# slobodaapl/nvit

Measured on AMD Instinct MI355X. Metric: images/sec (train step) nViT-B/16 224px, higher is better.
Workload: dtype bf16; 1 GPU; nViT-base 224px patches 8/16 T=784 C=768 L=12 H=12, full train step (fwd+bwd+clip+AdamW+renorm), synthetic images, formula weights; per_gpu_batch=128, global_batch=128, parallelism=dp1

## Files before the change

include/nvit_hip.h:

```cpp
#ifndef NVIT_HIP_H
#define NVIT_HIP_H
#include <stdint.h>

#ifdef __cplusplus
extern "C" {
#endif

#define NVIT_OK 0
#define NVIT_EINVAL 1001
#define NVIT_F32 0
#define NVIT_BF16 1
#define NVIT_BF16_F32IN 3

int nvit_version(void);
const char* nvit_last_error(void);

#define NVIT_KID_GEMM_NT 0
#define NVIT_KID_GEMM_TN 1
#define NVIT_KID_ATTN_FWD 2
#define NVIT_KID_ATTN_BWD 3
#define NVIT_KID_ROWOPS 4
#define NVIT_KID_RENORM 5
#define NVIT_KID_SHADOW 6
#define NVIT_KID_PATCHIFY 7
#define NVIT_KID_MISC 8
#define NVIT_KID_GEMM_F32 9
#define NVIT_KID_GEMM_SWIGLU 10
#define NVIT_KID_GEMM_QKNORM 11
#define NVIT_KID_GEMM_SWIGLU_BWD 12
#define NVIT_KID_OPTIM 13
#define NVIT_KID_GEMM_SWIGLU_ACT 14
#define NVIT_KID_COUNT 15
void nvit_prof_enable(int on);
void nvit_prof_select(unsigned mask);
int nvit_prof_collect(double* ms, double* flops, double* bytes, int64_t* launches);
const char* nvit_prof_name(int kid);

#define NVIT_RENORM_ROWS_PER_ITEM 64
#define NVIT_RENORM_COLS_PER_ITEM 64
#define NVIT_RENORM_TALL_ROWS 1152
#define NVIT_RENORM_TALL_COLS_PER_ITEM 32
#define NVIT_RENORM_MAX_ROWS_DIM0 2048
int nvit_renorm_weights(const int64_t* table, int n, int total_items, void* stream);

int nvit_shadow_weights(const int64_t* table, int n, int total_items, int dt, void* stream);

int nvit_adamw_tick(float* hyper, double beta1, double beta2, void* stream);
int nvit_grad_sqnorm(const int64_t* table, int n, int total_chunks, float* partial, int npart, void* stream);
int nvit_adamw_renorm(const int64_t* table, int n, int total_items, int max_slab_rows, float beta1, float beta2,
                      float eps, double bias_correction1, double bias_correction2, const float* partial, int npart,
                      float max_norm, float* gnorm_out, const float* hyper, void* stream);

int nvit_gemm_nt(int dt, const void* A, int lda, const void* B, int ldb, void* C, int ldc, int out_dt,
                 int M, int N, int K, const float* bias, const float* colscale, const float* rowadd,
                 int rowadd_period, int accumulate, void* stream);

int nvit_set_gemm_sched(int dynamic);
int nvit_set_gemm_impl(int nt_impl, int tn_impl);
int nvit_gemm_nt_fusable(int dt, int M, int N, int K);
int nvit_gemm_nt_swiglu_bwd(int dt, const void* A, int lda, const void* B, int ldb, const void* uv, void* duv,
                            float* part, int M, int F, int K, const float* gs, float gscale, void* stream);
int nvit_gemm_nt_swiglu(int dt, const void* A, int lda, const void* B, int ldb, void* uv, void* xm, int M, int F,
                        int K, const float* gs, float gscale, void* stream);
int nvit_gemm_nt_swiglu_act(int dt, const void* A, int lda, const void* B, int ldb, void* xm, int M, int F, int K,
                            const float* gs, float gscale, void* stream);
int nvit_gemm_nt_qknorm(int dt, const void* A, int lda, const void* B, int ldb, int M, int K, int nparts, int part0,
                        const float* sqk, float c_q, float q_prescale, void* qh, void* kh, void* vh, float* rq, float* rk,
                        int T, int H, int d, void* stream);
int nvit_gemm_nt_swiglu_bias(int dt, const void* A, int lda, const void* B, int ldb, void* uv, void* xm, int M, int F,
                             int K, const float* gs, float gscale, const float* bias, void* stream);
int nvit_gemm_nt_swiglu_act_bias(int dt, const void* A, int lda, const void* B, int ldb, void* xm, int M, int F, int K,
                                 const float* gs, float gscale, const float* bias, void* stream);
int nvit_gemm_nt_qknorm_bias(int dt, const void* A, int lda, const void* B, int ldb, int M, int K, int nparts, int part0,
                             const float* sqk, float c_q, float q_prescale, void* qh, void* kh, void* vh, float* rq,
                             float* rk, int T, int H, int d, const float* bias, void* stream);

int nvit_gemm_tn(int dt, const void* A, int lda, const void* B, int ldb, float* G, int ldg, int Mred, int N,
                 int K, int splits, float* ws, int64_t ws_bytes, int perm, int accumulate, void* stream);

int nvit_lerp_fwd(int dt, const float* h, const void* y, int y_dt, const float* alpha, float c_a,
                  const float* skip_x, const float* skip, float* out, void* out_lo, int M, int C, void* stream);
int nvit_lerp_bwd_blocks(int dt, int y_dt, int C, int has_add, int has_skip, int accum);
int nvit_lerp_bwd(int dt, const float* dout, const void* dout_add, const float* h, const void* y, int y_dt, const float* alpha,
                  float c_a, const float* skip_x, const float* skip, float* dh, int accum_dh, float* dy,
                  void* dy_lo, float* dskip_x, float* part_dlam, float* part_dskip, int nblk, int M, int C,
                  void* stream);

int nvit_rmsnorm_fwd(const float* x, const float* w, float eps, float* out, float* rstd, int M, int C, void* stream);
int nvit_rmsnorm_bwd(const float* dout, const float* x, const float* w, const float* rstd, float* dx, float* part_dw,
                     int nblk, int M, int C, void* stream);
int nvit_res_rmsnorm_fwd(int dt, const float* a, const void* y, int y_dt, const float* w, float eps, float* out,
                         void* out_lo, float* rstd, int M, int C, void* stream);
int nvit_res_rmsnorm_bwd(int dt, const float* g, const void* g_add, const float* a, const void* y, int y_dt,
                         const float* w, const float* rstd, float* dz, int accum, void* dz_lo, float* part_dw, int nblk,
                         int M, int C, void* stream);
int nvit_res_skip_fwd(int dt, const float* h, const void* y, int y_dt, const float* skip, const float* x, float* out,
                      void* out_lo, int M, int C, void* stream);
int nvit_res_skip_bwd(int dt, const float* dout, const float* h, const void* y, int y_dt, const float* skip,
                      const float* x, float* dh, void* dh_lo, float* dx, float* part_dskip, int nblk, int M, int C,
                      void* stream);
int nvit_norm_skip_fwd(const float* src, const float* tgt, const float* skip, float* out, int M, int C, void* stream);
int nvit_norm_skip_bwd(const float* dout, const float* src, const float* tgt, const float* skip, float* dsrc,
                       float* dtgt, float* part_dskip, int nblk, int M, int C, void* stream);

int nvit_qknorm_fwd(int dt, const void* q, int ldq, const void* k, int ldk, const void* v, int ldv,
                    const float* sqk, float c_q, void* qh, void* kh, void* vh, float* rq, float* rk, int B,
                    int T, int H, int d, void* stream);
int nvit_qknorm_bwd(int dt, const void* dqh, const void* dkh, const void* dvh, const void* qh, const void* kh,
                    const float* rq, const float* rk, const float* sqk, float c_q, void* dq, int ldq,
                    void* dk, int ldk, void* dv, int ldv, float* part_dsqk, int nblk, int B, int T, int H,
                    int d, void* stream);

int nvit_heads_pad_fwd(int dt, const float* q, int ldq, const float* k, int ldk, const float* v, int ldv,
                       const float* sqk, float c_q, void* qh, void* kh, void* vh, float* rq, float* rk,
                       float* sqk_pad, int B, int T, int H, int d, int dp, void* stream);
int nvit_heads_pad_bwd(int dt, const void* dqh, const void* dkh, const void* dvh, const void* qh, const void* kh,
                       const float* rq, const float* rk, const float* sqk, float c_q, void* dq, int ldq,
                       void* dk, int ldk, void* dv, int ldv, float* part_dsqk, int nblk, int B, int T, int H,
                       int d, int dp, void* stream);
int nvit_pad_cols(int dt, const void* src, void* dst, int M, int H, int d, int dp, void* stream);
int nvit_unpad_cols(int dt, const void* src, void* dst, int M, int H, int d, int dp, void* stream);

int nvit_swiglu_fwd(int dt, const void* uv, const float* suv, float gscale, void* x, int M, int F, void* stream);
int nvit_swiglu_bwd(int dt, const void* dx, const void* uv, const float* suv, float gscale, void* duv,
                    float* part_dsuv, int rows_per_blk, int M, int F, void* stream);

int nvit_colsum_reduce(const float* part, int nblk, int N, float* out, int accumulate, int kind, const float* ref,
                       float scale, void* stream);
int nvit_colsum_reduce_multi(const int64_t* part, const int* nblk, const int64_t* part_b, const int* nblk_b, const int* N,
                             const int64_t* out, const int* accumulate, const int* kind, const int64_t* ref,
                             const float* scale, int n, void* stream);
int nvit_colsum(const void* a, int a_dt, int lda, const void* b, int b_dt, int ldb, int R, int N, int period,
                float* out, int accumulate, float scale, void* stream);
int nvit_cast(const float* src, void* dst, int dt, int64_t n, void* stream);
int nvit_normalize_images(const void* in, int in_is_u8_hwc, float* out, int B, int C, int H, int W, float mean, float std_,
                          void* stream);
int nvit_scale_cols(const float* a, int lda, const float* s, float c, void* out, int out_dt, int ldo, int R, int N,
                    void* stream);

int nvit_attn_fwd(int dt, int impl, const void* qh, const void* kh, const void* vh, float scale, void* o, float* lse,
                  int B, int H, int Tq, int Tk, int d, void* stream);
int nvit_attn_fwd_bounded(int dt, int impl, const void* qh, const void* kh, const void* vh, float scale, const float* sqk,
                          float c_q, float q_prescale, void* o, float* lse, int B, int H, int Tq, int Tk, int d,
                          void* stream);
int nvit_attn_bwd(int dt, int impl, const void* dout, const void* qh, const void* kh, const void* vh, const void* o,
                  const float* lse, float scale, void* dqh, void* dkh, void* dvh, float* delta, int B, int H,
                  int Tq, int Tk, int d, void* stream);

int nvit_attn_bwd_qknorm(int dt, const void* dout, const void* qh, const void* kh, const void* vh, const void* o,
                         const float* lse, float scale, const float* rq, const float* rk, const float* sqk, float c_q,
                         float q_prescale, void* dq, int ldq, void* dk, void* dv, int ldkv, float* part_q, float* part_k,
                         float* delta, int B, int H, int Tq, int Tk, int d, void* stream);

#define NVIT_ATTN_HEADS_MAX_H 32
int nvit_attn_heads_fwd(int dt, const float* q, int ldq, const float* k, const float* v, int ldkv, const float* sqk,
                        float c_q, float scale, void* o, float* lse, int M, int H, int d, void* stream);
int nvit_attn_heads_bwd(int dt, const void* dout, const float* q, int ldq, const float* k, const float* v, int ldkv,
                        const float* sqk, float c_q, float scale, const float* lse, void* dq, int lddq, void* dk,
                        void* dv, int lddkv, float* part_dsqk, int nblk, int M, int H, int d, void* stream);

int nvit_im2col(int dt, const float* img, void* A_l, void* A_g, int B, int ch, int S, int Pl, int Pg, void* stream);
int nvit_patch_embed_kp(int K);
int nvit_patch_embed_fwd(const float* img, const void* w_l, const float* b_l, const float* pos_l, float* out_l, void* lo_l,
                         void* a_l, const void* w_g, const float* b_g, const float* pos_g, float* out_g, void* lo_g,
                         void* a_g, int B, int ch, int S, int Pl, int Pg, int C, void* stream);
int nvit_pool_ln_fwd(int dt, const float* x, const float* w, const float* b, float eps, float* pooled, float* ln,
                     void* ln_lo, float* stats, float* ws, int nchunk, int B, int T, int C, void* stream);
int nvit_pool_ln_bwd(const float* dln, const float* pooled, const float* w, const float* stats, float* dx,
                     float* dw, float* db, int accumulate, int B, int T, int C, void* stream);
int nvit_recon_loss(const float* raw, const float* img, float* part, int nblk, float* loss, int B, int ch, int S,
                    int P, void* stream);

int nvit_som_bmu(const float* scores, const float* nodes, float* nn_ws, int64_t M, int N, int C, int64_t* idx,
                 void* stream);
int nvit_gather_rows(const float* nodes, const int64_t* idx, float* out, int64_t M, int C, void* stream);
int nvit_scatter_rows(const float* dout, const int64_t* idx, float* dnodes, int64_t M, int N, int C, void* stream);
int nvit_onehot(const int64_t* idx, float* out, int64_t M, int N, void* stream);
int nvit_som_update(float* nodes, const float* x, const int64_t* idx, float lr_alpha, float sigma, int gm, int gn,
                    int periodic, float* v_ws, float* s_ws, int B, int T, int C, void* stream);
int nvit_som_update_dev(float* nodes, const float* x, const int64_t* idx, const float* lr_alpha, float sigma, int gm,
                        int gn, int periodic, float* v_ws, float* s_ws, int B, int T, int C, void* stream);
int nvit_cos_consistency_fwd(const float* a, const float* b, float* stats, float* part, int nblk, float* loss,
                             int64_t M, int C, void* stream);
int nvit_cos_consistency_bwd(const float* a, const float* b, const float* stats, const float* g, float* da, float* db,
                             int64_t M, int C, void* stream);
int nvit_huber_fwd(const float* a, const float* b, float* part, int nblk, float* loss, int64_t n, void* stream);
int nvit_huber_bwd(const float* a, const float* b, const float* g, float* da, float* db, int64_t n, void* stream);
int nvit_som_smooth_fwd(const float* nodes, const int64_t* idx, int* cnt, float* D, float* loss, int64_t M, int Nn,
                        int C, int map_size, void* stream);
int nvit_som_smooth_bwd(const float* nodes, const float* D, const int* cnt, const float* g, float* dnodes,
                        int accumulate, int64_t M, int Nn, int C, int map_size, void* stream);
int nvit_recon_bwd(int dt, const float* raw, const float* img, const float* g, void* draw, int B, int ch, int S, int P,
                   void* stream);

int nvit_ce_loss(const float* logits, const int64_t* labels, float* rowloss, float* loss, float* dlogits, int B, int N,
                 void* stream);
int nvit_eval_metrics(const float* logits, const int64_t* labels, float* acc, int B, int N, void* stream);

int64_t nvit_xgmi_chunk(int64_t n, int nranks);
int nvit_xgmi_reduce_scatter(const int64_t* peer_ptrs, int nranks, int rank, int64_t n, float scale, void* stream);
int nvit_xgmi_all_gather(const int64_t* peer_ptrs, int nranks, int rank, int64_t n, void* stream);

int64_t nvit_xgmi_flag_bytes(int nslots);
int nvit_xgmi_flags_alloc(int nslots, void** dev_ptr, void* ipc_handle_out);
int nvit_xgmi_flags_open(const void* ipc_handle, void** dev_ptr);
int nvit_xgmi_flags_close(void* dev_ptr);
int nvit_xgmi_flags_free(void* dev_ptr);
int nvit_xgmi_flags_error(const void* own_flags, int nslots, unsigned* out, void* stream);
int nvit_xgmi_reduce_scatter_sync(const int64_t* peer_ptrs, const int64_t* flag_ptrs, int nranks, int rank, int nslots,
                                  int slot, unsigned epoch, int64_t off, int64_t n, float scale, void* stream);
int nvit_xgmi_all_gather_sync(const int64_t* peer_ptrs, const int64_t* flag_ptrs, int nranks, int rank, int nslots, int slot,
                              unsigned epoch, int64_t off, int64_t n, void* stream);
int nvit_xgmi_wait_gathered(const int64_t* flag_ptrs, int nranks, int rank, int nslots, const int* slots,
                            const unsigned* epochs, int nwait, void* host_err_dev, void* stream);
int nvit_xgmi_set_timeout(double seconds);
int nvit_xgmi_errword_alloc(void** host_ptr, void** dev_ptr);
int nvit_xgmi_errword_free(void* host_ptr);

int nvit_set_attn_dkv_asm(int on);

#ifdef __cplusplus
}
#endif
#endif
```

nvit_amd/_lib.py:

```python
from __future__ import annotations

import ctypes as C
import os

_HERE = os.path.dirname(os.path.abspath(__file__))
LIB_PATH = os.environ.get("NVIT_LIB") or os.path.join(_HERE, "libnvit_hip.so")

F32, BF16, BF16_F32IN = 0, 1, 3
KID_NAMES = ["gemm_nt", "gemm_tn", "attn_fwd", "attn_bwd", "rowops", "renorm", "shadow", "patchify", "misc", "gemm_f32",
             "gemm_swiglu", "gemm_qknorm", "gemm_swiglu_bwd", "optim", "gemm_swiglu_act"]
RENORM_ROWS_PER_ITEM = 64
RENORM_COLS_PER_ITEM = 64
RENORM_TALL_ROWS = 1152
RENORM_TALL_COLS_PER_ITEM = 32
RENORM_MAX_ROWS_DIM0 = 2048
MAX_EMBD = 2048
ATTN_HEADS_MAX_H = 32

_vp, _i, _f, _i64 = C.c_void_p, C.c_int, C.c_float, C.c_int64

SIGNATURES = {
    "nvit_version": [],
    "nvit_last_error": [],
    "nvit_prof_enable": [_i],
    "nvit_prof_select": [C.c_uint],
    "nvit_prof_collect": [_vp, _vp, _vp, _vp],
    "nvit_prof_name": [_i],
    "nvit_renorm_weights": [_vp, _i, _i, _vp],
    "nvit_shadow_weights": [_vp, _i, _i, _i, _vp],
    "nvit_grad_sqnorm": [_vp, _i, _i, _vp, _i, _vp],
    "nvit_adamw_renorm": [_vp, _i, _i, _i, _f, _f, _f, C.c_double, C.c_double, _vp, _i, _f, _vp, _vp, _vp],
    "nvit_adamw_tick": [_vp, C.c_double, C.c_double, _vp],
    "nvit_set_gemm_sched": [_i],
    "nvit_set_gemm_impl": [_i, _i],
    "nvit_ce_loss": [_vp, _vp, _vp, _vp, _vp, _i, _i, _vp],
    "nvit_eval_metrics": [_vp, _vp, _vp, _i, _i, _vp],
    "nvit_gemm_nt": [_i, _vp, _i, _vp, _i, _vp, _i, _i, _i, _i, _i, _vp, _vp, _vp, _i, _i, _vp],
    "nvit_gemm_nt_fusable": [_i, _i, _i, _i],
    "nvit_gemm_nt_swiglu": [_i, _vp, _i, _vp, _i, _vp, _vp, _i, _i, _i, _vp, _f, _vp],
    "nvit_gemm_nt_swiglu_act": [_i, _vp, _i, _vp, _i, _vp, _i, _i, _i, _vp, _f, _vp],
    "nvit_gemm_nt_swiglu_bwd": [_i, _vp, _i, _vp, _i, _vp, _vp, _vp, _i, _i, _i, _vp, _f, _vp],
    "nvit_gemm_nt_qknorm": [_i, _vp, _i, _vp, _i, _i, _i, _i, _i, _vp, _f, _f, _vp, _vp, _vp, _vp, _vp, _i, _i, _i, _vp],
    "nvit_gemm_nt_swiglu_bias": [_i, _vp, _i, _vp, _i, _vp, _vp, _i, _i, _i, _vp, _f, _vp, _vp],
    "nvit_gemm_nt_swiglu_act_bias": [_i, _vp, _i, _vp, _i, _vp, _i, _i, _i, _vp, _f, _vp, _vp],
    "nvit_gemm_nt_qknorm_bias": [_i, _vp, _i, _vp, _i, _i, _i, _i, _i, _vp, _f, _f, _vp, _vp, _vp, _vp, _vp, _i, _i, _i, _vp,
                                 _vp],
    "nvit_gemm_tn": [_i, _vp, _i, _vp, _i, _vp, _i, _i, _i, _i, _i, _vp, _i64, _i, _i, _vp],
    "nvit_lerp_fwd": [_i, _vp, _vp, _i, _vp, _f, _vp, _vp, _vp, _vp, _i, _i, _vp],
    "nvit_lerp_bwd_blocks": [_i, _i, _i, _i, _i, _i],
    "nvit_lerp_bwd": [_i, _vp, _vp, _vp, _vp, _i, _vp, _f, _vp, _vp, _vp, _i, _vp, _vp, _vp, _vp, _vp, _i, _i, _i, _vp],
    "nvit_norm_skip_fwd": [_vp, _vp, _vp, _vp, _i, _i, _vp],
    "nvit_norm_skip_bwd": [_vp, _vp, _vp, _vp, _vp, _vp, _vp, _i, _i, _i, _vp],
    "nvit_qknorm_fwd": [_i, _vp, _i, _vp, _i, _vp, _i, _vp, _f, _vp, _vp, _vp, _vp, _vp, _i, _i, _i, _i, _vp],
    "nvit_qknorm_bwd": [_i, _vp, _vp, _vp, _vp, _vp, _vp, _vp, _vp, _f, _vp, _i, _vp, _i, _vp, _i, _vp, _i, _i, _i,
                        _i, _i, _vp],
    "nvit_heads_pad_fwd": [_i, _vp, _i, _vp, _i, _vp, _i, _vp, _f, _vp, _vp, _vp, _vp, _vp, _vp, _i, _i, _i, _i, _i, _vp],
    "nvit_heads_pad_bwd": [_i, _vp, _vp, _vp, _vp, _vp, _vp, _vp, _vp, _f, _vp, _i, _vp, _i, _vp, _i, _vp, _i, _i, _i,
                           _i, _i, _i, _vp],
    "nvit_pad_cols": [_i, _vp, _vp, _i, _i, _i, _i, _vp],
    "nvit_unpad_cols": [_i, _vp, _vp, _i, _i, _i, _i, _vp],
    "nvit_swiglu_fwd": [_i, _vp, _vp, _f, _vp, _i, _i, _vp],
    "nvit_swiglu_bwd": [_i, _vp, _vp, _vp, _f, _vp, _vp, _i, _i, _i, _vp],
    "nvit_colsum_reduce_multi": [_vp, _vp, _vp, _vp, _vp, _vp, _vp, _vp, _vp, _vp, _i, _vp],
    "nvit_colsum_reduce": [_vp, _i, _i, _vp, _i, _i, _vp, _f, _vp],
    "nvit_colsum": [_vp, _i, _i, _vp, _i, _i, _i, _i, _i, _vp, _i, _f, _vp],
    "nvit_cast": [_vp, _vp, _i, _i64, _vp],
    "nvit_normalize_images": [_vp, _i, _vp, _i, _i, _i, _i, _f, _f, _vp],
    "nvit_scale_cols": [_vp, _i, _vp, _f, _vp, _i, _i, _i, _i, _vp],
    "nvit_attn_fwd": [_i, _i, _vp, _vp, _vp, _f, _vp, _vp, _i, _i, _i, _i, _i, _vp],
    "nvit_attn_fwd_bounded": [_i, _i, _vp, _vp, _vp, _f, _vp, _f, _f, _vp, _vp, _i, _i, _i, _i, _i, _vp],
    "nvit_attn_bwd": [_i, _i, _vp, _vp, _vp, _vp, _vp, _vp, _f, _vp, _vp, _vp, _vp, _i, _i, _i, _i, _i, _vp],
    "nvit_attn_bwd_qknorm": [_i, _vp, _vp, _vp, _vp, _vp, _vp, _f, _vp, _vp, _vp, _f, _f, _vp, _i, _vp, _vp, _i, _vp, _vp,
                             _vp, _i, _i, _i, _i, _i, _vp],
    "nvit_attn_heads_fwd": [_i, _vp, _i, _vp, _vp, _i, _vp, _f, _f, _vp, _vp, _i, _i, _i, _vp],
    "nvit_attn_heads_bwd": [_i, _vp, _vp, _i, _vp, _vp, _i, _vp, _f, _f, _vp, _vp, _i, _vp, _vp, _i, _vp, _i, _i, _i, _i,
                            _vp],
    "nvit_im2col": [_i, _vp, _vp, _vp, _i, _i, _i, _i, _i, _vp],
    "nvit_patch_embed_kp": [_i],
    "nvit_patch_embed_fwd": [_vp, _vp, _vp, _vp, _vp, _vp, _vp, _vp, _vp, _vp, _vp, _vp, _vp, _i, _i, _i, _i, _i, _i, _vp],
    "nvit_pool_ln_fwd": [_i, _vp, _vp, _vp, _f, _vp, _vp, _vp, _vp, _vp, _i, _i, _i, _i, _vp],
    "nvit_pool_ln_bwd": [_vp, _vp, _vp, _vp, _vp, _vp, _vp, _i, _i, _i, _i, _vp],
    "nvit_som_bmu": [_vp, _vp, _vp, _i64, _i, _i, _vp, _vp],
    "nvit_gather_rows": [_vp, _vp, _vp, _i64, _i, _vp],
    "nvit_scatter_rows": [_vp, _vp, _vp, _i64, _i, _i, _vp],
    "nvit_onehot": [_vp, _vp, _i64, _i, _vp],
    "nvit_rmsnorm_fwd": [_vp, _vp, _f, _vp, _vp, _i, _i, _vp],
    "nvit_rmsnorm_bwd": [_vp, _vp, _vp, _vp, _vp, _vp, _i, _i, _i, _vp],
    "nvit_res_rmsnorm_fwd": [_i, _vp, _vp, _i, _vp, _f, _vp, _vp, _vp, _i, _i, _vp],
    "nvit_res_rmsnorm_bwd": [_i, _vp, _vp, _vp, _vp, _i, _vp, _vp, _vp, _i, _vp, _vp, _i, _i, _i, _vp],
    "nvit_res_skip_fwd": [_i, _vp, _vp, _i, _vp, _vp, _vp, _vp, _i, _i, _vp],
    "nvit_res_skip_bwd": [_i, _vp, _vp, _vp, _i, _vp, _vp, _vp, _vp, _vp, _vp, _i, _i, _i, _vp],
    "nvit_som_update": [_vp, _vp, _vp, _f, _f, _i, _i, _i, _vp, _vp, _i, _i, _i, _vp],
    "nvit_som_update_dev": [_vp, _vp, _vp, _vp, _f, _i, _i, _i, _vp, _vp, _i, _i, _i, _vp],
    "nvit_cos_consistency_fwd": [_vp, _vp, _vp, _vp, _i, _vp, _i64, _i, _vp],
    "nvit_cos_consistency_bwd": [_vp, _vp, _vp, _vp, _vp, _vp, _i64, _i, _vp],
    "nvit_huber_fwd": [_vp, _vp, _vp, _i, _vp, _i64, _vp],
    "nvit_huber_bwd": [_vp, _vp, _vp, _vp, _vp, _i64, _vp],
    "nvit_som_smooth_fwd": [_vp, _vp, _vp, _vp, _vp, _i64, _i, _i, _i, _vp],
    "nvit_som_smooth_bwd": [_vp, _vp, _vp, _vp, _vp, _i, _i64, _i, _i, _i, _vp],
    "nvit_recon_bwd": [_i, _vp, _vp, _vp, _vp, _i, _i, _i, _i, _vp],
    "nvit_recon_loss": [_vp, _vp, _vp, _i, _vp, _i, _i, _i, _i, _vp],
    "nvit_xgmi_chunk": [_i64, _i],
    "nvit_xgmi_reduce_scatter": [_vp, _i, _i, _i64, _f, _vp],
    "nvit_xgmi_all_gather": [_vp, _i, _i, _i64, _vp],
    "nvit_xgmi_flag_bytes": [_i],
    "nvit_xgmi_flags_alloc": [_i, _vp, _vp],
    "nvit_xgmi_flags_open": [_vp, _vp],
    "nvit_xgmi_flags_close": [_vp],
    "nvit_xgmi_flags_free": [_vp],
    "nvit_xgmi_flags_error": [_vp, _i, _vp, _vp],
    "nvit_xgmi_reduce_scatter_sync": [_vp, _vp, _i, _i, _i, _i, C.c_uint, _i64, _i64, _f, _vp],
    "nvit_xgmi_all_gather_sync": [_vp, _vp, _i, _i, _i, _i, C.c_uint, _i64, _i64, _vp],
    "nvit_xgmi_wait_gathered": [_vp, _i, _i, _i, _vp, _vp, _i, _vp, _vp],
    "nvit_xgmi_set_timeout": [C.c_double],
    "nvit_xgmi_errword_alloc": [_vp, _vp],
    "nvit_xgmi_errword_free": [_vp],
    "nvit_set_attn_dkv_asm": [_i],
}
_RESTYPES = {"nvit_last_error": C.c_char_p, "nvit_prof_name": C.c_char_p, "nvit_prof_enable": None, "nvit_prof_select": None,
             "nvit_xgmi_chunk": C.c_int64, "nvit_xgmi_flag_bytes": C.c_int64}

_lib = None


def load() -> C.CDLL:
    global _lib
    if _lib is not None:
        return _lib
    if not os.path.exists(LIB_PATH):
        raise RuntimeError(
            f"nvit_amd: {LIB_PATH} not found. Build it with `python -c 'import __graft_entry__ as g; g.build()'` "
            "(hipcc --offload-arch=gfx950). There is no CPU fallback for the nViT hot path.")
    lib = C.CDLL(LIB_PATH)
    for name, args in SIGNATURES.items():
        fn = getattr(lib, name)
        fn.argtypes = args
        fn.restype = _RESTYPES.get(name, C.c_int)
    _lib = lib
    return lib


def check(rc: int, what: str) -> None:
    if rc != 0:
        msg = load().nvit_last_error()
        raise RuntimeError(f"{what} failed (code {rc}): {msg.decode() if msg else ''}")
```

nvit_amd/csrc/gemm_p.hip:

```cpp
#include "gemm_common.h"

namespace {

template <int FM>
struct PCfg;
template <>
struct PCfg<4> {
  static constexpr int PBM = 256, PBN = 128, WR = 4, WC = 2, NSLOT = 3, A_DMA = 4, B_DMA = 2;
};
template <>
struct PCfg<8> {
  static constexpr int PBM = 256, PBN = 256, WR = 2, WC = 4, NSLOT = 2, A_DMA = 4, B_DMA = 4;
};

template <int N>
__device__ __forceinline__ void wait_vmcnt() {
  static_assert(N >= 0 && N < 64, "vmcnt is a 6-bit counter");
  asm volatile("s_waitcnt vmcnt(%0)" ::"n"(N) : "memory");
}

template <typename T, int FM, int EPI, bool DYN>
__global__ __launch_bounds__(512) void gemm_nt_persistent_kernel(NtArgs g, int tiles_m, int ntiles, unsigned* sched) {
  using Cfg = PCfg<FM>;
  constexpr int PBM = Cfg::PBM, PBN = Cfg::PBN, NSLOT = Cfg::NSLOT;
  constexpr int A_BYTES = PBM * ROWB, B_BYTES = PBN * ROWB, SLOT_BYTES = A_BYTES + B_BYTES;
  constexpr int DPS = Cfg::A_DMA + Cfg::B_DMA;
  constexpr int WROWS = 16 * FM;
  constexpr int NST = EPI == 1 ? 2 * FM : EPI == 2 ? 4 * FM : EPI == 3 ? 3 * FM : EPI == 4 ? 2 * FM : EPI == 5 ? 8 : EPI == 6 ? FM : 0;
  extern __shared__ __attribute__((aligned(16))) char smem[];
  constexpr int EPC = 16 / sizeof(T);
  constexpr int BK = ROWB / sizeof(T);
  const int tid = threadIdx.x, lane = tid & 63;
  const int wid = __builtin_amdgcn_readfirstlane(tid >> 6);
  const int wr = wid / Cfg::WC, wc = wid % Cfg::WC;
  const int l15 = lane & 15, lg = lane >> 4;
  const int nt = g.K / BK;
  const int G = gridDim.x;
  const int slot_in_round = (blockIdx.x & 7) * (G >> 3) + (blockIdx.x >> 3);
  const int my_tiles = slot_in_round < ntiles ? (ntiles - slot_in_round + G - 1) / G : 0;
  const int total_stages = my_tiles * nt;
  const int xcd = blockIdx.x & 7, Gx = G >> 3;
  const int x_start = (int)(((long long)ntiles * xcd) >> 3);
  const int x_len = (int)(((long long)ntiles * (xcd + 1)) >> 3) - x_start;
  const int first_tile = (int)(blockIdx.x >> 3) < x_len ? x_start + (int)(blockIdx.x >> 3) : -1;
  int* s_next = reinterpret_cast<int*>(smem + NSLOT * SLOT_BYTES + 8 * 2048);
  auto sched_exit = [&]() {
    if (tid == 0) {
      if (atomicAdd(&sched[8], 1u) == (unsigned)(G - 1)) {
#pragma unroll
        for (int i = 0; i < 9; ++i) sched[i] = 0u;
      }
    }
  };
  if constexpr (DYN) {
    if (first_tile < 0) {
      sched_exit();
      return;
    }
  } else {
    if (total_stages == 0) return;
  }

  const int srow = lane >> 3;
  const int gc = (lane & 7) ^ srow;
  const unsigned lds_base = (unsigned)(uintptr_t)((__attribute__((address_space(3))) void*)smem);
  const unsigned wave_off = (unsigned)(wid * 1024);

  auto tile_of = [&](int pid, int& m0, int& n0) {
    constexpr int GM = 8;
    const int per_group = GM * g.tiles_n;
    const int group = pid / per_group, first_m = group * GM;
    const int gsz = (tiles_m - first_m) < GM ? (tiles_m - first_m) : GM;
    const int in_g = pid - group * per_group;
    m0 = (first_m + in_g % gsz) * PBM;
    n0 = (in_g / gsz) * PBN;
  };

  const bool loader = wid < 4;
  unsigned aoff[2][Cfg::A_DMA], boff[2][Cfg::B_DMA];
  unsigned long long abase = 0, bbase = 0;
  int l_it = 0, l_k = 0, l_slot = 0;
  bool l_valid = true;
  int pending_c = -1;
  int c_tile = DYN ? first_tile : slot_in_round;
  int wraps = 0;
  unsigned ticket = 0;
  int ticket_age = -1;
  constexpr int PUBLISH_AGE = 3;
  auto draw = [&]() {
    if (tid == 0) ticket = atomicAdd(&sched[xcd], 1u);
    ticket_age = 0;
  };
  auto publish = [&]() {
    if (ticket_age >= 0 && ++ticket_age > PUBLISH_AGE) {
      if (tid == 0) {
        const long long idx = (long long)Gx + ticket;
        s_next[wraps & 1] = idx < x_len ? x_start + (int)idx : -1;
      }
      ticket_age = -1;
    }
  };
  auto set_load_tile = [&](int pid) {
    int m0, n0;
    tile_of(pid, m0, n0);
    if (loader) {
#pragma unroll
      for (int h = 0; h < 2; ++h) {
        const int w = wid + 4 * h;
#pragma unroll
        for (int i = 0; i < Cfg::A_DMA; ++i) {
          int ra = m0 + (i * 8 + w) * 8 + srow;
          ra = ra < g.M ? ra : g.M - 1;
          aoff[h][i] = (unsigned)(((size_t)(ra - m0) * g.lda + (size_t)gc * EPC) * sizeof(T));
        }
#pragma unroll
        for (int i = 0; i < Cfg::B_DMA; ++i) {
          int rb = n0 + (i * 8 + w) * 8 + srow;
          rb = rb < g.N ? rb : g.N - 1;
          boff[h][i] = (unsigned)(((size_t)(rb - n0) * g.ldb + (size_t)gc * EPC) * sizeof(T));
        }
      }
    }
    abase = (unsigned long long)(uintptr_t)g.A + (unsigned long long)((size_t)m0 * g.lda * sizeof(T));
    bbase = (unsigned long long)(uintptr_t)g.B + (unsigned long long)((size_t)n0 * g.ldb * sizeof(T));
  };
  auto issue_stage = [&]() {
    const unsigned bo = lds_base + wave_off + (unsigned)l_slot * SLOT_BYTES;
    const size_t ko = (size_t)l_k * ROWB;
    {
      if (loader) {
        glds16s_n<Cfg::A_DMA>(abase + ko, aoff[0], bo);
        glds16s_n<Cfg::A_DMA>(abase + ko, aoff[1], bo + 4096);
        glds16s_n<Cfg::B_DMA>(bbase + ko, boff[0], bo + A_BYTES);
        glds16s_n<Cfg::B_DMA>(bbase + ko, boff[1], bo + A_BYTES + 4096);
      }
    }
    l_slot = l_slot == NSLOT - 1 ? 0 : l_slot + 1;
    if (++l_k == nt) {
      l_k = 0;
      if constexpr (DYN) {
        const int nxt = __builtin_amdgcn_readfirstlane(s_next[wraps & 1]);
        ++wraps;
        pending_c = nxt;
        if (nxt >= 0) {
          set_load_tile(nxt);
          draw();
        } else {
          l_valid = false;
        }
      } else {
        ++l_it;
        if (l_it < my_tiles) set_load_tile(l_it * G + slot_in_round);
      }
    }
  };

  f32x4 acc[FM][4];
#pragma unroll
  for (int i = 0; i < FM; ++i)
#pragma unroll
    for (int j = 0; j < 4; ++j) acc[i][j] = (f32x4){0.f, 0.f, 0.f, 0.f};

#define LOAD_FRAGS(FA, FB, slot_, kk_)                                                          \
  {                                                                                             \
    const char* la_ = smem + (slot_) * SLOT_BYTES;                                              \
    const char* lb_ = la_ + A_BYTES;                                                            \
    const int c_ = (kk_) * 4 + lg;                                                              \
    _Pragma("unroll") for (int i = 0; i < FM; ++i) {                                            \
      const int r = wr * WROWS + i * 16 + l15;                                                  \
      FA[i] = *reinterpret_cast<const uint4*>(la_ + r * ROWB + ((c_ ^ (r & 7)) << 4));          \
    }                                                                                           \
    _Pragma("unroll") for (int j = 0; j < 4; ++j) {                                             \
      const int r = wc * 64 + j * 16 + l15;                                                     \
      FB[j] = *reinterpret_cast<const uint4*>(lb_ + r * ROWB + ((c_ ^ (r & 7)) << 4));          \
    }                                                                                           \
  }
#define MMA_FRAGS(FA, FB)                                                                       \
  _Pragma("unroll") for (int i = 0; i < FM; ++i) _Pragma("unroll") for (int j = 0; j < 4; ++j)  \
      Mma<T>::run(FB[j], FA[i], acc[i][j]);

  set_load_tile(c_tile);
  if constexpr (DYN) draw();
  issue_stage();
  const bool two_ahead = NSLOT > 2 && (DYN || total_stages > 1);
  if (two_ahead) issue_stage();
  if (two_ahead && loader)
    wait_vmcnt<(NSLOT > 2 ? 2 * DPS : 0)>();
  else
    wait_vmcnt<0>();
  __syncthreads();

  int c_it = 0, c_k = 0;
  int slot = 0;
  for (int s = 0;; ++s) {
    const bool issued_now = DYN ? l_valid : (s + NSLOT - 1 < total_stages);
    if (issued_now) issue_stage();
    {
      const char* la_ = smem + slot * SLOT_BYTES;
      const char* lb_ = la_ + A_BYTES;
      uint4 fa[2][FM], fb[2][4];
#define RA(kk_, i_)                                                                                       \
  {                                                                                                       \
    const int r = wr * WROWS + (i_) * 16 + l15;                                                           \
    fa[kk_][i_] = *reinterpret_cast<const uint4*>(la_ + r * ROWB + ((((kk_) * 4 + lg) ^ (r & 7)) << 4));  \
  }
#define RB(kk_, j_)                                                                                       \
  {                                                                                                       \
    const int r = wc * 64 + (j_) * 16 + l15;                                                              \
    fb[kk_][j_] = *reinterpret_cast<const uint4*>(lb_ + r * ROWB + ((((kk_) * 4 + lg) ^ (r & 7)) << 4));  \
  }
      __builtin_amdgcn_sched_barrier(0);
      RB(0, 0) RB(0, 1) RB(0, 2) RB(0, 3) RA(0, 0) RA(0, 1) RA(0, 2)
      if constexpr (FM == 8) {
        RA(0, 3) RB(1, 0) RA(0, 4) RB(1, 1) RA(0, 5) RB(1, 2) RA(0, 6) RB(1, 3) RA(0, 7)
        RA(1, 0) RA(1, 1) RA(1, 2) RA(1, 3) RA(1, 4) RA(1, 5) RA(1, 6) RA(1, 7)
      } else {
        RA(0, 3) RB(1, 0) RB(1, 1) RB(1, 2) RB(1, 3) RA(1, 0) RA(1, 1) RA(1, 2) RA(1, 3)
      }
#pragma unroll
      for (int kk = 0; kk < 2; ++kk)
#pragma unroll
        for (int i = 0; i < FM; ++i)
#pragma unroll
          for (int j = 0; j < 4; ++j) Mma<T>::run(fb[kk][j], fa[kk][i], acc[i][j]);
      constexpr int MPS = sizeof(T) == 2 ? 4 : 16;
      __builtin_amdgcn_sched_group_barrier(0x100, 7, 0);
#pragma unroll
      for (int t = 0; t < 2 * FM; ++t) {
        __builtin_amdgcn_sched_group_barrier(0x8, MPS, 0);
        if constexpr (FM == 8) {
          if (t < 4)
            __builtin_amdgcn_sched_group_barrier(0x100, 2, 0);
          else if (t < 13)
            __builtin_amdgcn_sched_group_barrier(0x100, 1, 0);
        } else {
          if (t < 3)
            __builtin_amdgcn_sched_group_barrier(0x100, 2, 0);
          else if (t < 6)
            __builtin_amdgcn_sched_group_barrier(0x100, 1, 0);
        }
      }
      __builtin_amdgcn_sched_barrier(0);
#undef RA
#undef RB
    }
    bool stored = false, full_tile = false, more = true;
    if (++c_k == nt) {
      int m0, n0;
      tile_of(c_tile, m0, n0);
      full_tile = NST > 0 && m0 + PBM <= g.M && n0 + PBN <= g.N;
      {
        char* scratch = smem + NSLOT * SLOT_BYTES + wid * 2048;
        if constexpr (EPI == 1)
          nt_store_tile_staged<FM, bf16>(g, acc, m0 + wr * WROWS, n0 + wc * 64, lane, scratch);
        else if constexpr (EPI == 2)
          nt_store_tile_staged<FM, float>(g, acc, m0 + wr * WROWS, n0 + wc * 64, lane, scratch);
        else if constexpr (EPI == 3)
          nt_store_tile_swiglu<FM>(g, acc, m0 + wr * WROWS, n0 + wc * 64, lane, scratch);
        else if constexpr (EPI == 4)
          nt_store_tile_qknorm<FM>(g, acc, m0 + wr * WROWS, n0 + wc * 64, lane, scratch);
        else if constexpr (EPI == 5)
          nt_store_tile_swiglu_bwd<FM>(g, acc, m0 + wr * WROWS, n0 + wc * 64, lane, scratch);
        else if constexpr (EPI == 6)
          nt_store_tile_swiglu<FM, false>(g, acc, m0 + wr * WROWS, n0 + wc * 64, lane, scratch);
        else
          nt_store_tile<FM>(g, acc, m0 + wr * WROWS, n0 + wc * 64, l15, lg);
      }
#pragma unroll
      for (int i = 0; i < FM; ++i)
#pragma unroll
        for (int j = 0; j < 4; ++j) acc[i][j] = (f32x4){0.f, 0.f, 0.f, 0.f};
      c_k = 0;
      stored = true;
      if constexpr (DYN) {
        c_tile = pending_c;
        more = c_tile >= 0;
      } else {
        ++c_it;
        c_tile = c_it * G + slot_in_round;
        more = c_it < my_tiles;
      }
    }
    if constexpr (DYN) publish();
    if (stored) {
      if (full_tile && issued_now) {
        if (loader)
          wait_vmcnt<(NSLOT - 2) * 2 * DPS + NST>();
        else
          wait_vmcnt<NST>();
      } else {
        wait_vmcnt<0>();
      }
    } else if (NSLOT > 2 && issued_now && loader) {
      wait_vmcnt<(NSLOT > 2 ? (NSLOT - 2) * 2 * DPS : 0)>();
    } else {
      wait_vmcnt<0>();
    }
    if (!more) break;
    __syncthreads();
    slot = slot == NSLOT - 1 ? 0 : slot + 1;
  }
  if constexpr (DYN) sched_exit();
#undef LOAD_FRAGS
#undef MMA_FRAGS
}

__device__ unsigned nvit_sched_slots[64][16];
bool g_gemm_sched_dynamic = false;

unsigned* sched_slot() {
  static void* base[NVIT_MAX_DEVICES] = {};
  static unsigned next = 0;
  unsigned* p = (unsigned*)nvit_symbol_address(HIP_SYMBOL(nvit_sched_slots), base);
  return p ? p + 16 * (next++ & 63) : nullptr;
}

template <typename T, int FM, int EPI>
int launch_p2(const NtArgs& g_in, int n_cu, hipStream_t s) {
  using Cfg = PCfg<FM>;
  constexpr int LDS_STATIC = Cfg::NSLOT * (Cfg::PBM + Cfg::PBN) * ROWB + 8 * 2048;
  constexpr bool CAN_DYN = LDS_STATIC + 16 <= 160 * 1024;
  constexpr int LDS_BYTES = CAN_DYN ? LDS_STATIC + 16 : LDS_STATIC;
  static bool attr_set = false;
  if (!attr_set) {
    hipError_t e = hipFuncSetAttribute((const void*)gemm_nt_persistent_kernel<T, FM, EPI, false>,
                                       hipFuncAttributeMaxDynamicSharedMemorySize, LDS_BYTES);
    if (e == hipSuccess && CAN_DYN)
      e = hipFuncSetAttribute((const void*)gemm_nt_persistent_kernel<T, FM, EPI, CAN_DYN>,
                              hipFuncAttributeMaxDynamicSharedMemorySize, LDS_BYTES);
    if (e != hipSuccess) NVIT_FAIL((int)e, "gemm_nt: cannot raise LDS limit: %s", hipGetErrorString(e));
    attr_set = true;
  }
  NtArgs g = g_in;
  g.tiles_n = cdiv(g.N, Cfg::PBN);
  const int tiles_m = cdiv(g.M, Cfg::PBM);
  const int nt = g.K / (ROWB / (int)sizeof(T));
  unsigned* sched = (CAN_DYN && g_gemm_sched_dynamic && nt >= Cfg::NSLOT + 4) ? sched_slot() : nullptr;
  if (sched)
    hipLaunchKernelGGL((gemm_nt_persistent_kernel<T, FM, EPI, CAN_DYN>), dim3(n_cu), dim3(512), LDS_BYTES, s, g, tiles_m,
                       tiles_m * g.tiles_n, sched);
  else
    hipLaunchKernelGGL((gemm_nt_persistent_kernel<T, FM, EPI, false>), dim3(n_cu), dim3(512), LDS_BYTES, s, g, tiles_m,
                       tiles_m * g.tiles_n, (unsigned*)nullptr);
  NVIT_CHECK_LAUNCH("gemm_nt_persistent");
  return NVIT_OK;
}

template <typename T, int FM>
int launch_p(const NtArgs& g, int n_cu, hipStream_t s) {
  const int eo = g.out_dt == NVIT_F32 ? 4 : 8;
  const bool staged = (g.N % eo) == 0 && (g.ldc % eo) == 0;
  if (!staged) return launch_p2<T, FM, 0>(g, n_cu, s);
  return g.out_dt == NVIT_F32 ? launch_p2<T, FM, 2>(g, n_cu, s) : launch_p2<T, FM, 1>(g, n_cu, s);
}

}

static int p_num_cu() {
  int n = nvit_num_cu();
  if (n == 0) return 0;
  n -= n % 8;
  return n < 8 ? 8 : n;
}

extern "C" int nvit_set_gemm_sched(int dynamic) {
  g_gemm_sched_dynamic = dynamic != 0;
  return NVIT_OK;
}

int nvit_gemm_nt_fused_launch(const NtArgs& g, int epi, hipStream_t s) {
  const int n_cu = p_num_cu();
  if (n_cu == 0) NVIT_FAIL(NVIT_EINVAL, "gemm_nt: cannot query device properties");
  if (epi == 5) return launch_p2<bf16, 8, 5>(g, n_cu, s);
  if (epi == 6) return launch_p2<bf16, 8, 6>(g, n_cu, s);
  return epi == 3 ? launch_p2<bf16, 8, 3>(g, n_cu, s) : launch_p2<bf16, 8, 4>(g, n_cu, s);
}

int nvit_gemm_nt_persistent_launch(int dt, const NtArgs& g, int tile_n, hipStream_t s) {
  const int n_cu = p_num_cu();
  if (n_cu == 0) NVIT_FAIL(NVIT_EINVAL, "gemm_nt: cannot query device properties");
  if (dt == NVIT_BF16) return tile_n == 256 ? launch_p<bf16, 8>(g, n_cu, s) : launch_p<bf16, 4>(g, n_cu, s);
  return tile_n == 256 ? launch_p<float, 8>(g, n_cu, s) : launch_p<float, 4>(g, n_cu, s);
}
```

Baseline: 1300 images/sec.

## Use shorter M tiles for the tail wave of persistent NT GEMM

Adds a short-tile plan for the persistent 256x256 NT GEMM. When the tile count leaves a partial final wave, the remaining rows are covered with shorter tiles (32*FMS rows) so that the tail fits within one wave of workgroups. This targets wave quantization and tail imbalance across CUs. In exchange it adds more template instantiations and a second loop phase, and the short tiles run at lower MMA efficiency.

Result: no change. 1298 images/sec (-0.1%).

```diff
diff --git a/include/nvit_hip.h b/include/nvit_hip.h
--- a/include/nvit_hip.h
+++ b/include/nvit_hip.h
@@ -56,6 +56,8 @@
                  int rowadd_period, int accumulate, void* stream);
 
 int nvit_set_gemm_sched(int dynamic);
+int nvit_set_gemm_nt_short_tile(int on);
+int nvit_gemm_nt_short_plan(int M, int N, int n_wg, int* plan);
 int nvit_set_gemm_impl(int nt_impl, int tn_impl);
 int nvit_gemm_nt_fusable(int dt, int M, int N, int K);
 int nvit_gemm_nt_swiglu_bwd(int dt, const void* A, int lda, const void* B, int ldb, const void* uv, void* duv,
diff --git a/nvit_amd/_lib.py b/nvit_amd/_lib.py
--- a/nvit_amd/_lib.py
+++ b/nvit_amd/_lib.py
@@ -32,6 +32,8 @@
     "nvit_adamw_renorm": [_vp, _i, _i, _i, _f, _f, _f, C.c_double, C.c_double, _vp, _i, _f, _vp, _vp, _vp],
     "nvit_adamw_tick": [_vp, C.c_double, C.c_double, _vp],
     "nvit_set_gemm_sched": [_i],
+    "nvit_set_gemm_nt_short_tile": [_i],
+    "nvit_gemm_nt_short_plan": [_i, _i, _i, _vp],
     "nvit_set_gemm_impl": [_i, _i],
     "nvit_ce_loss": [_vp, _vp, _vp, _vp, _vp, _i, _i, _vp],
     "nvit_eval_metrics": [_vp, _vp, _vp, _i, _i, _vp],
diff --git a/nvit_amd/csrc/gemm_p.hip b/nvit_amd/csrc/gemm_p.hip
--- a/nvit_amd/csrc/gemm_p.hip
+++ b/nvit_amd/csrc/gemm_p.hip
@@ -1,3 +1,5 @@
+#include <type_traits>
+
 #include "gemm_common.h"
 
 namespace {
@@ -19,8 +21,81 @@
   asm volatile("s_waitcnt vmcnt(%0)" ::"n"(N) : "memory");
 }
 
-template <typename T, int FM, int EPI, bool DYN>
-__global__ __launch_bounds__(512) void gemm_nt_persistent_kernel(NtArgs g, int tiles_m, int ntiles, unsigned* sched) {
+template <int F>
+__device__ constexpr int p_reads_after(int t) {
+  if (F == 4) return t < 3 ? 2 : t < 6 ? 1 : 0;
+  constexpr int twos = F < 4 ? F : 4;
+  return t < twos ? 2 : t < twos + (2 * F + 1 - 2 * twos) ? 1 : 0;
+}
+template <typename T, int F, int FA>
+__device__ __forceinline__ void p_stage_mma(const char* la_, const char* lb_, int arow0, int brow0, int l15, int lg,
+                                            f32x4 (&acc)[FA][4]) {
+  static_assert(F >= 2 && F <= FA, "fragment rows of the stage body");
+  uint4 fa[2][F], fb[2][4];
+#define RA(kk_, i_)                                                                                       \
+  {                                                                                                       \
+    const int r = arow0 + (i_) * 16 + l15;                                                                \
+    fa[kk_][i_] = *reinterpret_cast<const uint4*>(la_ + r * ROWB + ((((kk_) * 4 + lg) ^ (r & 7)) << 4));  \
+  }
+#define RB(kk_, j_)                                                                                       \
+  {                                                                                                       \
+    const int r = brow0 + (j_) * 16 + l15;                                                                \
+    fb[kk_][j_] = *reinterpret_cast<const uint4*>(lb_ + r * ROWB + ((((kk_) * 4 + lg) ^ (r & 7)) << 4));  \
+  }
+  __builtin_amdgcn_sched_barrier(0);
+  if constexpr (F == 8) {
+    RB(0, 0) RB(0, 1) RB(0, 2) RB(0, 3) RA(0, 0) RA(0, 1) RA(0, 2)
+    RA(0, 3) RB(1, 0) RA(0, 4) RB(1, 1) RA(0, 5) RB(1, 2) RA(0, 6) RB(1, 3) RA(0, 7)
+    RA(1, 0) RA(1, 1) RA(1, 2) RA(1, 3) RA(1, 4) RA(1, 5) RA(1, 6) RA(1, 7)
+  } else if constexpr (F == 4) {
+    RB(0, 0) RB(0, 1) RB(0, 2) RB(0, 3) RA(0, 0) RA(0, 1) RA(0, 2)
+    RA(0, 3) RB(1, 0) RB(1, 1) RB(1, 2) RB(1, 3) RA(1, 0) RA(1, 1) RA(1, 2) RA(1, 3)
+  } else {
+#pragma unroll
+    for (int kk = 0; kk < 2; ++kk) {
+#pragma unroll
+      for (int j = 0; j < 4; ++j) RB(kk, j)
+#pragma unroll
+      for (int i = 0; i < F; ++i) RA(kk, i)
+    }
+  }
+#pragma unroll
+  for (int kk = 0; kk < 2; ++kk)
+#pragma unroll
+    for (int i = 0; i < F; ++i)
+#pragma unroll
+      for (int j = 0; j < 4; ++j) Mma<T>::run(fb[kk][j], fa[kk][i], acc[i][j]);
+  constexpr int MPS = sizeof(T) == 2 ? 4 : 16;
+  __builtin_amdgcn_sched_group_barrier(0x100, 7, 0);
+#pragma unroll
+  for (int t = 0; t < 2 * F; ++t) {
+    __builtin_amdgcn_sched_group_barrier(0x8, MPS, 0);
+    if constexpr (F == 8) {
+      if (t < 4)
+        __builtin_amdgcn_sched_group_barrier(0x100, 2, 0);
+      else if (t < 13)
+        __builtin_amdgcn_sched_group_barrier(0x100, 1, 0);
+    } else if constexpr (F == 4) {
+      if (t < 3)
+        __builtin_amdgcn_sched_group_barrier(0x100, 2, 0);
+      else if (t < 6)
+        __builtin_amdgcn_sched_group_barrier(0x100, 1, 0);
+    } else {
+      if (p_reads_after<F>(t) == 2)
+        __builtin_amdgcn_sched_group_barrier(0x100, 2, 0);
+      else if (p_reads_after<F>(t) == 1)
+        __builtin_amdgcn_sched_group_barrier(0x100, 1, 0);
+    }
+  }
+  __builtin_amdgcn_sched_barrier(0);
+#undef RA
+#undef RB
+}
+
+template <typename T, int FM, int EPI, bool DYN, int FMS = 0>
+__global__ __launch_bounds__(512) void gemm_nt_persistent_kernel(NtArgs g, int tiles_m, int ntiles, unsigned* sched,
+                                                                 int nfull, int tiles_ms) {
+  static_assert(FMS == 0 || (FM == 8 && !DYN && (EPI == 1 || EPI == 2) && FMS < FM), "short tiles: static 256x256 only");
   using Cfg = PCfg<FM>;
   constexpr int PBM = Cfg::PBM, PBN = Cfg::PBN, NSLOT = Cfg::NSLOT;
   constexpr int A_BYTES = PBM * ROWB, B_BYTES = PBN * ROWB, SLOT_BYTES = A_BYTES + B_BYTES;
@@ -66,13 +141,23 @@
   const unsigned lds_base = (unsigned)(uintptr_t)((__attribute__((address_space(3))) void*)smem);
   const unsigned wave_off = (unsigned)(wid * 1024);
 
-  auto tile_of = [&](int pid, int& m0, int& n0) {
+  auto tile_of = [&](int pid, int& m0, int& n0, int& rows) {
     constexpr int GM = 8;
+    int tm = tiles_m, h = PBM, mfirst = 0;
+    if constexpr (FMS > 0) {
+      if (pid >= nfull) {
+        pid -= nfull;
+        tm = tiles_ms;
+        h = 32 * FMS;
+        mfirst = tiles_m * PBM;
+      }
+    }
     const int per_group = GM * g.tiles_n;
     const int group = pid / per_group, first_m = group * GM;
-    const int gsz = (tiles_m - first_m) < GM ? (tiles_m - first_m) : GM;
+    const int gsz = (tm - first_m) < GM ? (tm - first_m) : GM;
     const int in_g = pid - group * per_group;
-    m0 = (first_m + in_g % gsz) * PBM;
+    m0 = mfirst + (first_m + in_g % gsz) * h;
+    rows = h;
     n0 = (in_g / gsz) * PBN;
   };
 
@@ -101,8 +186,8 @@
     }
   };
   auto set_load_tile = [&](int pid) {
-    int m0, n0;
-    tile_of(pid, m0, n0);
+    int m0, n0, rows;
+    tile_of(pid, m0, n0, rows);
     if (loader) {
 #pragma unroll
       for (int h = 0; h < 2; ++h) {
@@ -110,6 +195,7 @@
 #pragma unroll
         for (int i = 0; i < Cfg::A_DMA; ++i) {
           int ra = m0 + (i * 8 + w) * 8 + srow;
+          if constexpr (FMS > 0) ra = ra < m0 + rows ? ra : m0 + rows - 1;
           ra = ra < g.M ? ra : g.M - 1;
           aoff[h][i] = (unsigned)(((size_t)(ra - m0) * g.lda + (size_t)gc * EPC) * sizeof(T));
         }
@@ -191,65 +277,27 @@
   __syncthreads();
 
   int c_it = 0, c_k = 0;
-  int slot = 0;
-  for (int s = 0;; ++s) {
+  int slot = 0, s = 0;
+  auto run_stage = [&](auto fc) __attribute__((always_inline)) -> bool {
+    constexpr int F = decltype(fc)::value;
     const bool issued_now = DYN ? l_valid : (s + NSLOT - 1 < total_stages);
     if (issued_now) issue_stage();
     {
       const char* la_ = smem + slot * SLOT_BYTES;
-      const char* lb_ = la_ + A_BYTES;
-      uint4 fa[2][FM], fb[2][4];
-#define RA(kk_, i_)                                                                                       \
-  {                                                                                                       \
-    const int r = wr * WROWS + (i_) * 16 + l15;                                                           \
-    fa[kk_][i_] = *reinterpret_cast<const uint4*>(la_ + r * ROWB + ((((kk_) * 4 + lg) ^ (r & 7)) << 4));  \
-  }
-#define RB(kk_, j_)                                                                                       \
-  {                                                                                                       \
-    const int r = wc * 64 + (j_) * 16 + l15;                                                              \
-    fb[kk_][j_] = *reinterpret_cast<const uint4*>(lb_ + r * ROWB + ((((kk_) * 4 + lg) ^ (r & 7)) << 4));  \
-  }
-      __builtin_amdgcn_sched_barrier(0);
-      RB(0, 0) RB(0, 1) RB(0, 2) RB(0, 3) RA(0, 0) RA(0, 1) RA(0, 2)
-      if constexpr (FM == 8) {
-        RA(0, 3) RB(1, 0) RA(0, 4) RB(1, 1) RA(0, 5) RB(1, 2) RA(0, 6) RB(1, 3) RA(0, 7)
-        RA(1, 0) RA(1, 1) RA(1, 2) RA(1, 3) RA(1, 4) RA(1, 5) RA(1, 6) RA(1, 7)
-      } else {
-        RA(0, 3) RB(1, 0) RB(1, 1) RB(1, 2) RB(1, 3) RA(1, 0) RA(1, 1) RA(1, 2) RA(1, 3)
-      }
-#pragma unroll
-      for (int kk = 0; kk < 2; ++kk)
-#pragma unroll
-        for (int i = 0; i < FM; ++i)
-#pragma unroll
-          for (int j = 0; j < 4; ++j) Mma<T>::run(fb[kk][j], fa[kk][i], acc[i][j]);
-      constexpr int MPS = sizeof(T) == 2 ? 4 : 16;
-      __builtin_amdgcn_sched_group_barrier(0x100, 7, 0);
-#pragma unroll
-      for (int t = 0; t < 2 * FM; ++t) {
-        __builtin_amdgcn_sched_group_barrier(0x8, MPS, 0);
-        if constexpr (FM == 8) {
-          if (t < 4)
-            __builtin_amdgcn_sched_group_barrier(0x100, 2, 0);
-          else if (t < 13)
-            __builtin_amdgcn_sched_group_barrier(0x100, 1, 0);
-        } else {
-          if (t < 3)
-            __builtin_amdgcn_sched_group_barrier(0x100, 2, 0);
-          else if (t < 6)
-            __builtin_amdgcn_sched_group_barrier(0x100, 1, 0);
-        }
-      }
-      __builtin_amdgcn_sched_barrier(0);
-#undef RA
-#undef RB
+      p_stage_mma<T, F>(la_, la_ + A_BYTES, wr * 16 * F, wc * 64, l15, lg, acc);
     }
     bool stored = false, full_tile = false, more = true;
     if (++c_k == nt) {
-      int m0, n0;
-      tile_of(c_tile, m0, n0);
+      int m0, n0, rows;
+      tile_of(c_tile, m0, n0, rows);
       full_tile = NST > 0 && m0 + PBM <= g.M && n0 + PBN <= g.N;
-      {
+      if constexpr (F != FM) {
+        full_tile = false;
+        char* scratch = smem + NSLOT * SLOT_BYTES + wid * 2048;
+        using TO = std::conditional_t<EPI == 1, bf16, float>;
+        nt_store_tile_staged<F, TO>(g, reinterpret_cast<f32x4(&)[F][4]>(acc), m0 + wr * 16 * F, n0 + wc * 64, lane,
+                                    scratch);
+      } else {
         char* scratch = smem + NSLOT * SLOT_BYTES + wid * 2048;
         if constexpr (EPI == 1)
           nt_store_tile_staged<FM, bf16>(g, acc, m0 + wr * WROWS, n0 + wc * 64, lane, scratch);
@@ -296,9 +344,19 @@
     } else {
       wait_vmcnt<0>();
     }
-    if (!more) break;
+    if (!more) return false;
     __syncthreads();
     slot = slot == NSLOT - 1 ? 0 : slot + 1;
+    ++s;
+    return true;
+  };
+  if constexpr (FMS > 0) {
+    bool more = true;
+    while (more && c_tile < nfull) more = run_stage(std::integral_constant<int, FM>{});
+    while (more) more = run_stage(std::integral_constant<int, FMS>{});
+  } else {
+    while (run_stage(std::integral_constant<int, FM>{})) {
+    }
   }
   if constexpr (DYN) sched_exit();
 #undef LOAD_FRAGS
@@ -313,6 +371,55 @@
   static unsigned next = 0;
   unsigned* p = (unsigned*)nvit_symbol_address(HIP_SYMBOL(nvit_sched_slots), base);
   return p ? p + 16 * (next++ & 63) : nullptr;
+}
+
+constexpr int SHORT_FMS[] = {2, 3, 4, 5, 6, 7};
+bool g_gemm_nt_short_tile = true;
+
+struct ShortPlan {
+  int full;
+  int panels_full;
+  int rows_left;
+  int fms;
+  int tiles_short;
+};
+
+ShortPlan nt_short_plan(int M, int N, int G) {
+  ShortPlan p = {0, 0, 0, 0, 0};
+  if (M <= 0 || N <= 0 || G <= 0) return p;
+  const long long tiles_m = cdiv(M, 256), tiles_n = cdiv(N, 256), T = tiles_m * tiles_n;
+  p.full = (int)(T / G);
+  p.panels_full = (int)tiles_m;
+  if (T % G == 0 || p.full == 0) return p;
+  p.panels_full = (int)((long long)p.full * G / tiles_n);
+  p.rows_left = M - 256 * p.panels_full;
+  for (int fms : SHORT_FMS) {
+    const long long n = (long long)cdiv(p.rows_left, 32 * fms) * tiles_n;
+    if (n <= G) {
+      p.fms = fms;
+      p.tiles_short = (int)n;
+      return p;
+    }
+  }
+  p.panels_full = (int)tiles_m;
+  p.rows_left = 0;
+  return p;
+}
+
+template <typename T, int EPI, int FMS>
+int launch_short(const NtArgs& g, int n_cu, int lds_bytes, const ShortPlan& p, hipStream_t s) {
+  static bool attr_set = false;
+  if (!attr_set) {
+    const hipError_t e = hipFuncSetAttribute((const void*)gemm_nt_persistent_kernel<T, 8, EPI, false, FMS>,
+                                             hipFuncAttributeMaxDynamicSharedMemorySize, lds_bytes);
+    if (e != hipSuccess) NVIT_FAIL((int)e, "gemm_nt: cannot raise LDS limit: %s", hipGetErrorString(e));
+    attr_set = true;
+  }
+  const int nfull = p.panels_full * g.tiles_n;
+  hipLaunchKernelGGL((gemm_nt_persistent_kernel<T, 8, EPI, false, FMS>), dim3(n_cu), dim3(512), lds_bytes, s, g,
+                     p.panels_full, nfull + p.tiles_short, (unsigned*)nullptr, nfull, p.tiles_short / g.tiles_n);
+  NVIT_CHECK_LAUNCH("gemm_nt_persistent");
+  return NVIT_OK;
 }
 
 template <typename T, int FM, int EPI>
@@ -336,12 +443,27 @@
   const int tiles_m = cdiv(g.M, Cfg::PBM);
   const int nt = g.K / (ROWB / (int)sizeof(T));
   unsigned* sched = (CAN_DYN && g_gemm_sched_dynamic && nt >= Cfg::NSLOT + 4) ? sched_slot() : nullptr;
+  if constexpr (FM == 8 && (EPI == 1 || EPI == 2)) {
+    if (!sched && g_gemm_nt_short_tile) {
+      const ShortPlan p = nt_short_plan(g.M, g.N, n_cu);
+      switch (p.fms) {
+        case 2: return launch_short<T, EPI, 2>(g, n_cu, LDS_BYTES, p, s);
+        case 3: return launch_short<T, EPI, 3>(g, n_cu, LDS_BYTES, p, s);
+        case 4: return launch_short<T, EPI, 4>(g, n_cu, LDS_BYTES, p, s);
+        case 5: return launch_short<T, EPI, 5>(g, n_cu, LDS_BYTES, p, s);
+        case 6: return launch_short<T, EPI, 6>(g, n_cu, LDS_BYTES, p, s);
+        case 7: return launch_short<T, EPI, 7>(g, n_cu, LDS_BYTES, p, s);
+        default: break;
+      }
+    }
+  }
+  const int ntiles = tiles_m * g.tiles_n;
   if (sched)
     hipLaunchKernelGGL((gemm_nt_persistent_kernel<T, FM, EPI, CAN_DYN>), dim3(n_cu), dim3(512), LDS_BYTES, s, g, tiles_m,
-                       tiles_m * g.tiles_n, sched);
+                       ntiles, sched, ntiles, 0);
   else
     hipLaunchKernelGGL((gemm_nt_persistent_kernel<T, FM, EPI, false>), dim3(n_cu), dim3(512), LDS_BYTES, s, g, tiles_m,
-                       tiles_m * g.tiles_n, (unsigned*)nullptr);
+                       ntiles, (unsigned*)nullptr, ntiles, 0);
   NVIT_CHECK_LAUNCH("gemm_nt_persistent");
   return NVIT_OK;
 }
@@ -368,6 +490,20 @@
   return NVIT_OK;
 }
 
+extern "C" int nvit_set_gemm_nt_short_tile(int on) {
+  g_gemm_nt_short_tile = on != 0;
+  return NVIT_OK;
+}
+
+extern "C" int nvit_gemm_nt_short_plan(int M, int N, int n_wg, int* plan) {
+  NVIT_REQUIRE(plan != nullptr && M > 0 && N > 0 && n_wg >= 0, "gemm_nt_short_plan: bad arguments");
+  if (n_wg == 0) n_wg = p_num_cu();
+  if (n_wg == 0) NVIT_FAIL(NVIT_EINVAL, "gemm_nt: cannot query device properties");
+  const ShortPlan p = nt_short_plan(M, N, n_wg);
+  plan[0] = p.full, plan[1] = p.panels_full, plan[2] = p.rows_left, plan[3] = p.fms, plan[4] = p.tiles_short;
+  return p.fms > 0 ? 1 : 0;
+}
+
 int nvit_gemm_nt_fused_launch(const NtArgs& g, int epi, hipStream_t s) {
   const int n_cu = p_num_cu();
   if (n_cu == 0) NVIT_FAIL(NVIT_EINVAL, "gemm_nt: cannot query device properties");
```
